# lucidrains/phenaki-pytorch

Hardware: NVIDIA H100
Metric: cvivit_encode_frames_per_s (higher is better)
Workload: dtype bf16

## Files before the change

phenaki_pytorch_b200/csrc/gemm_wgmma.cu:

```cuda
#include "phk_common.cuh"
#include "phk_sm90.cuh"
#include <mutex>
#include <unordered_map>

namespace phk {

constexpr int GM = 128;
constexpr int GN = 128;
constexpr int GK = 64;
constexpr int GSTAGES = 4;
constexpr int EPI_WARPS = 16;
constexpr int GTHREADS = 128 + EPI_WARPS * 32;
constexpr int STAGE_BYTES = GM * GK * 2;
constexpr int CPAD = 132;
constexpr int CSTAGE_BYTES = GM * CPAD * 4;
constexpr int RING_BYTES = GSTAGES * 2 * STAGE_BYTES;
constexpr int SMEM_TOTAL = RING_BYTES + CSTAGE_BYTES + 256  + 1024 ;

struct EpiParams {
  void* C; int64_t ldc; int64_t M; int N; int K;
  const float* bias; const float* residual;
  int64_t seg_len, seg_stride, seg_off;
  int m_tiles, n_tiles;
  int tma_epi;
  const float* nscale; int norm_cols; float nmul;
  alignas(64) CUtensorMap tmC;
};


__device__ __forceinline__ void epi_bar_sync() { asm volatile("bar.sync 1, %0;" ::"n"(EPI_WARPS * 32) : "memory"); }

template <bool BOX>
__device__ __forceinline__ void acc_to_stage(const float (&d)[32], uint8_t* stage, int rq, int cq, int w, int lane,
                                             bool add) {
  const int r0 = rq + 16 * w + (lane >> 2);
#pragma unroll
  for (int j = 0; j < 8; ++j) {
    const int c = cq + 8 * j + 2 * (lane & 3);
#pragma unroll
    for (int h = 0; h < 2; ++h) {
      const int r = r0 + 8 * h;
      float2* dst = BOX ? reinterpret_cast<float2*>(stage + (c >> 5) * (GM * 128) + r * 128 +
                                                    ((((c & 31) >> 2) ^ (r & 7)) << 4) + (c & 3) * 4)
                        : reinterpret_cast<float2*>(reinterpret_cast<float*>(stage) + r * CPAD + c);
      float2 v = make_float2(d[4 * j + 2 * h], d[4 * j + 2 * h + 1]);
      if (add) { const float2 o = *dst; v.x += o.x; v.y += o.y; }
      *dst = v;
    }
  }
}

__device__ __forceinline__ float geglu_fast(float g, float v) {
  const float g2 = fminf(g * g, 64.0f);
  float u = fmaf(g2, -0.00035151678851506f, 0.037005646021930225f);
  u = fmaf(u, g2, 0.7975078842858219f);
  float t;
  asm("tanh.approx.f32 %0, %1;" : "=f"(t) : "f"(g * u));
  const float h = 0.5f * (g * v);
  return fmaf(h, t, h);
}


template <int EPI>
__device__ __forceinline__ bool epi_residual_prefetch(const EpiParams& p, float* cstage, int64_t m0, int n0, int ew,
                                                      int lane) {
  const bool res_vec = EPI == 0 && p.residual && (p.ldc % 4 == 0) && (p.N % 4 == 0) &&
                       ((reinterpret_cast<uintptr_t>(p.residual) & 15) == 0);
  if (res_vec) {
    const int col = n0 + lane * 4;
    const uint32_t seg_len = (uint32_t)p.seg_len;
#pragma unroll 1
    for (int rb = 0; rb < GM / EPI_WARPS; rb += 8) {
      float4 rv[8];
#pragma unroll
      for (int u = 0; u < 8; ++u) {
        const int r = (rb + u) * EPI_WARPS + ew;
        const uint32_t m = (uint32_t)m0 + r;
        uint32_t orow = m;
        if (seg_len > 0) { const uint32_t q = m / seg_len; orow = q * (uint32_t)p.seg_stride + (uint32_t)p.seg_off + (m - q * seg_len); }
        rv[u] = make_float4(0.f, 0.f, 0.f, 0.f);
        if (m < (uint32_t)p.M && col < p.N) rv[u] = *reinterpret_cast<const float4*>(p.residual + (int64_t)orow * p.ldc + col);
      }
#pragma unroll
      for (int u = 0; u < 8; ++u)
        *reinterpret_cast<float4*>(cstage + ((rb + u) * EPI_WARPS + ew) * CPAD + lane * 4) = rv[u];
    }
    epi_bar_sync();
  }
  return res_vec;
}

__device__ __forceinline__ void tma_store_2d(const CUtensorMap* map, uint32_t src, int c0, int c1) {
  asm volatile("cp.async.bulk.tensor.2d.global.shared::cta.bulk_group [%0, {%2, %3}], [%1];"
               ::"l"(map), "r"(src), "r"(c0), "r"(c1)
               : "memory");
}
__device__ __forceinline__ void tma_store_commit() { asm volatile("cp.async.bulk.commit_group;" ::: "memory"); }
__device__ __forceinline__ void tma_store_wait_read() { asm volatile("cp.async.bulk.wait_group.read 0;" ::: "memory"); }
__device__ __forceinline__ void tma_store_wait_all() { asm volatile("cp.async.bulk.wait_group 0;" ::: "memory"); }

__device__ __forceinline__ void epi_tma_begin(const EpiParams& p, uint32_t stage_s, uint32_t bar_res, int m0, int n0,
                                              int ew, int lane) {
  const bool store_thread = ew == 0 && lane == 0;
  if (store_thread) tma_store_wait_read();
  epi_bar_sync();
  if (p.residual && store_thread) {
    mbar_expect_tx(bar_res, 4 * GM * 128);
#pragma unroll
    for (int c = 0; c < 4; ++c) tma_load_2d(&p.tmC, bar_res, stage_s + c * (GM * 128), n0 + 32 * c, m0);
  }
}
__device__ __forceinline__ void epi_tma_finish(const EpiParams& p, uint8_t* stage, uint32_t stage_s, int m0, int n0,
                                               int ew, int lg, int part, int lane) {
  const int r = lg * 32 + lane;
  float4* box_row = reinterpret_cast<float4*>(stage + part * (GM * 128) + r * 128);
  const int col0 = n0 + part * 32;
  const bool bias_vec = p.bias && (col0 + 31 < p.N) && ((reinterpret_cast<uintptr_t>(p.bias) & 15) == 0);
#pragma unroll
  for (int j = 0; j < 8; ++j) {
    const int pos = j ^ (r & 7);
    float4 o = box_row[pos];
    if (bias_vec) {
      const float4 bv = __ldg(reinterpret_cast<const float4*>(p.bias + col0) + j);
      o.x += bv.x; o.y += bv.y; o.z += bv.z; o.w += bv.w;
    } else if (p.bias) {
      const int c = col0 + 4 * j;
      if (c < p.N) o.x += __ldg(p.bias + c);
      if (c + 1 < p.N) o.y += __ldg(p.bias + c + 1);
      if (c + 2 < p.N) o.z += __ldg(p.bias + c + 2);
      if (c + 3 < p.N) o.w += __ldg(p.bias + c + 3);
    }
    box_row[pos] = o;
  }
  asm volatile("fence.proxy.async.shared::cta;" ::: "memory");
  epi_bar_sync();
  if (ew == 0 && lane == 0) {
#pragma unroll
    for (int c = 0; c < 4; ++c)
      if (n0 + 32 * c < p.N) tma_store_2d(&p.tmC, stage_s + c * (GM * 128), n0 + 32 * c, m0);
    tma_store_commit();
  }
}

template <int EPI>
__device__ __forceinline__ void epi_chunk(const EpiParams& p, float* cstage, int64_t m0, int n0, bool res_vec, int ew,
                                          int lane) {
  const uint32_t seg_len = (uint32_t)p.seg_len;
  constexpr int RPW = GM / EPI_WARPS;
  const int ncol0 = n0;
  const int nlim = p.N;
  if (EPI == 0) {
    const int col = ncol0 + lane * 4;
    const bool vec = (p.ldc % 4 == 0) && ((reinterpret_cast<uintptr_t>(p.C) & 15) == 0) && (col + 3 < nlim);
    float4 bv = make_float4(0.f, 0.f, 0.f, 0.f);
    if (p.bias) {
      if (col < nlim) bv.x = __ldg(p.bias + col);
      if (col + 1 < nlim) bv.y = __ldg(p.bias + col + 1);
      if (col + 2 < nlim) bv.z = __ldg(p.bias + col + 2);
      if (col + 3 < nlim) bv.w = __ldg(p.bias + col + 3);
    }
    const bool fast = (p.ldc % 4 == 0) && ((reinterpret_cast<uintptr_t>(p.C) & 15) == 0) && (p.N % 4 == 0) &&
                      (res_vec || !p.residual) && (m0 + GM <= p.M) && seg_len == 0;
    if (fast) {
      if (col < nlim) {
        float* cbase = reinterpret_cast<float*>(p.C) + (m0 + ew) * p.ldc + col;
        const float* sbase = cstage + ew * CPAD + lane * 4;
#pragma unroll 1
        for (int rb = 0; rb < RPW; rb += 8) {
          float4 o[8];
#pragma unroll
          for (int u = 0; u < 8; ++u) o[u] = *reinterpret_cast<const float4*>(sbase + (rb + u) * EPI_WARPS * CPAD);
#pragma unroll
          for (int u = 0; u < 8; ++u) {
            o[u].x += bv.x; o[u].y += bv.y; o[u].z += bv.z; o[u].w += bv.w;
            *reinterpret_cast<float4*>(cbase + (int64_t)(rb + u) * EPI_WARPS * p.ldc) = o[u];
          }
        }
      }
    } else
#pragma unroll 1
    for (int rb = 0; rb < RPW; rb += 8) {
      int64_t off[8];
      float4 rv[8];
#pragma unroll
      for (int u = 0; u < 8; ++u) {
        const int r = (rb + u) * EPI_WARPS + ew;
        const uint32_t m = (uint32_t)m0 + r;
        uint32_t orow = m;
        if (seg_len > 0) { const uint32_t q = m / seg_len; orow = q * (uint32_t)p.seg_stride + (uint32_t)p.seg_off + (m - q * seg_len); }
        off[u] = (m < (uint32_t)p.M && col < nlim) ? (int64_t)orow * p.ldc + col : -1;
        rv[u] = make_float4(0.f, 0.f, 0.f, 0.f);
        if (!res_vec && vec && p.residual && off[u] >= 0) rv[u] = *reinterpret_cast<const float4*>(p.residual + off[u]);
      }
#pragma unroll
      for (int u = 0; u < 8; ++u) {
        if (off[u] < 0) continue;
        const int r = (rb + u) * EPI_WARPS + ew;
        float4 o = *reinterpret_cast<const float4*>(cstage + r * CPAD + lane * 4);
        o.x += bv.x + rv[u].x; o.y += bv.y + rv[u].y; o.z += bv.z + rv[u].z; o.w += bv.w + rv[u].w;
        float* crow = reinterpret_cast<float*>(p.C) + off[u];
        if (vec) {
          *reinterpret_cast<float4*>(crow) = o;
        } else {
          const float ov[4] = {o.x, o.y, o.z, o.w};
          for (int j = 0; j < 4; ++j)
            if (col + j < nlim) crow[j] = ov[j] + ((p.residual && !res_vec) ? p.residual[off[u] + j] : 0.f);
        }
      }
    }
  } else if (EPI == 3) {
    const int col = ncol0 + lane * 4;
    const bool norm = ncol0 < p.norm_cols;
    float4 sc = make_float4(1.f, 1.f, 1.f, 1.f);
    if (norm) {
      const float4 t = __ldg(reinterpret_cast<const float4*>(p.nscale + ((lane * 4) & 63)));
      sc = make_float4(t.x * p.nmul, t.y * p.nmul, t.z * p.nmul, t.w * p.nmul);
    }
#pragma unroll 4
    for (int rr = 0; rr < RPW; ++rr) {
      const int r = rr * EPI_WARPS + ew;
      const uint32_t m = (uint32_t)m0 + r;
      float4 o = *reinterpret_cast<const float4*>(cstage + r * CPAD + lane * 4);
      if (norm) {
        float ss = o.x * o.x + o.y * o.y + o.z * o.z + o.w * o.w;
#pragma unroll
        for (int d = 8; d > 0; d >>= 1) ss += __shfl_xor_sync(0xffffffffu, ss, d);
        const float inv = 1.0f / fmaxf(sqrtf(ss), 1e-12f);
        o.x = (o.x * inv) * sc.x; o.y = (o.y * inv) * sc.y; o.z = (o.z * inv) * sc.z; o.w = (o.w * inv) * sc.w;
      }
      if (m < (uint32_t)p.M && col < nlim)
        *reinterpret_cast<uint2*>(reinterpret_cast<__nv_bfloat16*>(p.C) + (int64_t)m * p.ldc + col) =
            make_uint2(pack_bf16x2(o.x, o.y), pack_bf16x2(o.z, o.w));
    }
  } else {
    constexpr int CPL = 4;
    const int col = ncol0 + lane * CPL;
    float bv[CPL];
#pragma unroll
    for (int j = 0; j < CPL; ++j) bv[j] = (p.bias && col + j < nlim) ? __ldg(p.bias + col + j) : 0.f;
    const bool vec = (p.ldc % CPL == 0) && ((reinterpret_cast<uintptr_t>(p.C) & 15) == 0) && (col + CPL - 1 < nlim);
#pragma unroll 4
    for (int rr = 0; rr < RPW; ++rr) {
      const int r = rr * EPI_WARPS + ew;
      const uint32_t m = (uint32_t)m0 + r;
      if (m >= (uint32_t)p.M) break;
      int64_t orow = m;
      if (seg_len > 0) { const uint32_t q = m / seg_len; orow = q * (uint32_t)p.seg_stride + (uint32_t)p.seg_off + (m - q * seg_len); }
      float o[CPL];
#pragma unroll
      for (int j = 0; j < CPL; ++j) o[j] = cstage[r * CPAD + lane * CPL + j] + bv[j];
      __nv_bfloat16* crow = reinterpret_cast<__nv_bfloat16*>(p.C) + orow * p.ldc + col;
      if (vec) {
        *reinterpret_cast<uint2*>(crow) = make_uint2(pack_bf16x2(o[0], o[1]), pack_bf16x2(o[2], o[3]));
      } else {
#pragma unroll
        for (int j = 0; j < CPL; ++j)
          if (col + j < nlim) crow[j] = __float2bfloat16_rn(o[j]);
      }
    }
  }
  epi_bar_sync();
}

template <int EPI, bool DUAL>
__global__ void __launch_bounds__(GTHREADS, 1) gemm_bf16_kernel(const __grid_constant__ CUtensorMap tmA,
                                                                const __grid_constant__ CUtensorMap tmB,
                                                                const __grid_constant__ EpiParams p,
                                                                const __grid_constant__ CUtensorMap tmA2,
                                                                const __grid_constant__ CUtensorMap tmB2,
                                                                const __grid_constant__ EpiParams p2) {
  pdl_trigger();
  extern __shared__ uint8_t smem_raw[];
  const uint32_t base = (smem_u32(smem_raw) + 1023u) & ~1023u;
  uint8_t* base_ptr = smem_raw + (base - smem_u32(smem_raw));
  const uint32_t sA = base, sB = base + GSTAGES * STAGE_BYTES;
  float* cstage = reinterpret_cast<float*>(base_ptr + RING_BYTES);
  const uint32_t bars = base + RING_BYTES + CSTAGE_BYTES;
  const uint32_t bar_res = bars + 16 * GSTAGES;
  const int warp = threadIdx.x >> 5, lane = threadIdx.x & 31;
  const int tiles1 = p.m_tiles * p.n_tiles;
  const int num_tiles = tiles1 + (DUAL ? p2.m_tiles * p2.n_tiles : 0);
  const int my_tiles = (int)blockIdx.x < num_tiles ? (num_tiles - 1 - (int)blockIdx.x) / (int)gridDim.x + 1 : 0;
  auto tile_of = [&](int i, int& m0, int& n0) -> bool {
    int tile = (int)blockIdx.x + i * (int)gridDim.x;
    const bool second = DUAL && tile >= tiles1;
    if (second) tile -= tiles1;
    const int mt = second ? p2.m_tiles : p.m_tiles;
    m0 = (tile % mt) * GM;
    n0 = (tile / mt) * GN;
    return second;
  };
  auto kblocks = [&](bool second) { return ((second ? p2.K : p.K) + GK - 1) / GK; };

  if (threadIdx.x == 0) {
    asm volatile("prefetch.tensormap [%0];" ::"l"(&tmA) : "memory");
    asm volatile("prefetch.tensormap [%0];" ::"l"(&tmB) : "memory");
    if (DUAL) {
      asm volatile("prefetch.tensormap [%0];" ::"l"(&tmA2) : "memory");
      asm volatile("prefetch.tensormap [%0];" ::"l"(&tmB2) : "memory");
    }
    for (int s = 0; s < GSTAGES; ++s) {
      mbar_init(bars + 8 * s, 1);
      mbar_init(bars + 8 * (GSTAGES + s), EPI_WARPS);
    }
    mbar_init(bar_res, 1);
    asm volatile("fence.mbarrier_init.release.cluster;" ::: "memory");
  }
  __syncthreads();
  pdl_wait();

  if (warp < 4) {
    if (warp == 0 && lane == 0) {
      int stage = 0;
      uint32_t phase = 0;
      for (int it = 0; it < my_tiles; ++it) {
        int m0, n0;
        const bool second = tile_of(it, m0, n0);
        const int num_kb = kblocks(second);
        const CUtensorMap* ma = second ? &tmA2 : &tmA;
        const CUtensorMap* mb = second ? &tmB2 : &tmB;
        for (int kb = 0; kb < num_kb; ++kb) {
          mbar_wait(bars + 8 * (GSTAGES + stage), phase ^ 1);
          const uint32_t full = bars + 8 * stage;
          mbar_expect_tx(full, 2 * STAGE_BYTES);
          tma_load_2d(ma, full, sA + stage * STAGE_BYTES, kb * GK, m0);
          tma_load_2d(mb, full, sB + stage * STAGE_BYTES, kb * GK, n0);
          if (++stage == GSTAGES) { stage = 0; phase ^= 1; }
        }
      }
    }
  } else {
    const int ew = warp - 4;
    const int lg = warp & 3;
    const int part = ew >> 2;
    const int wg = ew >> 2;
    const int rq = (wg & 1) * 64, cq = (wg >> 1) * 64;
    uint32_t res_phase = 0;
    int stage = 0;
    uint32_t phase = 0;
    for (int it = 0; it < my_tiles; ++it) {
      int m0, n0;
      const bool second = tile_of(it, m0, n0);
      const EpiParams& pp = second ? p2 : p;
      const bool tma = EPI == 0 && pp.tma_epi;
      bool res_vec = false;
      if (tma) epi_tma_begin(pp, base + RING_BYTES, bar_res, m0, n0, ew, lane);
      else if (EPI == 0) res_vec = epi_residual_prefetch<EPI>(pp, cstage, m0, n0, ew, lane);
      else epi_bar_sync();
      float d[32];
#pragma unroll
      for (int i = 0; i < 32; ++i) d[i] = 0.f;
      const int num_kb = kblocks(second);
      for (int kb = 0; kb < num_kb; ++kb) {
        mbar_wait(bars + 8 * stage, phase);
        const uint64_t da = gmma_desc(sA + stage * STAGE_BYTES + rq * 128);
        const uint64_t db = gmma_desc(sB + stage * STAGE_BYTES + cq * 128);
        wgmma_fence();
#pragma unroll
        for (int k = 0; k < GK / 16; ++k)
          wgmma_m64n64k16_ss<0>(d, da + 2 * k, db + 2 * k, 1u);
        wgmma_commit();
        wgmma_wait<0>();
        __syncwarp();
        if (lane == 0) mbar_arrive(bars + 8 * (GSTAGES + stage));
        if (++stage == GSTAGES) { stage = 0; phase ^= 1; }
      }
      if (tma) {
        if (pp.residual) { mbar_wait(bar_res, res_phase); res_phase ^= 1; }
        acc_to_stage<true>(d, reinterpret_cast<uint8_t*>(cstage), rq, cq, ew & 3, lane, pp.residual != nullptr);
      } else {
        acc_to_stage<false>(d, reinterpret_cast<uint8_t*>(cstage), rq, cq, ew & 3, lane, res_vec);
      }
      epi_bar_sync();
      if (tma)
        epi_tma_finish(pp, reinterpret_cast<uint8_t*>(cstage), base + RING_BYTES, m0, n0, ew, lg, part, lane);
      else
        epi_chunk<EPI>(pp, cstage, m0, n0, res_vec, ew, lane);
    }
    if (EPI == 0 && ew == 0 && lane == 0) tma_store_wait_read();
  }
  __syncthreads();
}

constexpr int GG_STAGES = 6;
constexpr int GG_THREADS = 384;
constexpr int GG_PRODUCER_REGS = 40, GG_CONSUMER_REGS = 232;
constexpr int GG_SMEM_TOTAL = GG_STAGES * 2 * STAGE_BYTES + 128  + 1024 ;
constexpr int GG_BAR_TURN = 1;

__global__ void __launch_bounds__(GG_THREADS, 1) gemm_bf16_geglu_kernel(const __grid_constant__ CUtensorMap tmA,
                                                                        const __grid_constant__ CUtensorMap tmB,
                                                                        const __grid_constant__ EpiParams p) {
  pdl_trigger();
  extern __shared__ uint8_t smem_raw[];
  const uint32_t base = (smem_u32(smem_raw) + 1023u) & ~1023u;
  const uint32_t sA = base, sB = base + GG_STAGES * STAGE_BYTES;
  const uint32_t bars = base + GG_STAGES * 2 * STAGE_BYTES;
  const int warp = threadIdx.x >> 5, lane = threadIdx.x & 31;
  const int num_tiles = p.m_tiles * p.n_tiles;
  const int my_tiles = (int)blockIdx.x < num_tiles ? (num_tiles - 1 - (int)blockIdx.x) / (int)gridDim.x + 1 : 0;
  const int num_kb = (p.K + GK - 1) / GK;
  auto tile_of = [&](int i, int& m0, int& n0) {
    const int tile = (int)blockIdx.x + i * (int)gridDim.x;
    m0 = (tile % p.m_tiles) * GM;
    n0 = (tile / p.m_tiles) * GN;
  };

  if (threadIdx.x == 0) {
    asm volatile("prefetch.tensormap [%0];" ::"l"(&tmA) : "memory");
    asm volatile("prefetch.tensormap [%0];" ::"l"(&tmB) : "memory");
    for (int s = 0; s < GG_STAGES; ++s) {
      mbar_init(bars + 8 * s, 1);
      mbar_init(bars + 8 * (GG_STAGES + s), 4);
    }
    asm volatile("fence.mbarrier_init.release.cluster;" ::: "memory");
  }
  __syncthreads();
  pdl_wait();

  if (warp < 4) {
    setmaxnreg_dec<GG_PRODUCER_REGS>();
    if (warp == 0 && lane == 0) {
      int stage = 0;
      uint32_t phase = 0;
      for (int it = 0; it < my_tiles; ++it) {
        int m0, n0;
        tile_of(it, m0, n0);
        for (int kb = 0; kb < num_kb; ++kb) {
          mbar_wait(bars + 8 * (GG_STAGES + stage), phase ^ 1);
          const uint32_t full = bars + 8 * stage;
          mbar_expect_tx(full, 2 * STAGE_BYTES);
          tma_load_2d(&tmA, full, sA + stage * STAGE_BYTES, kb * GK, m0);
          tma_load_2d(&tmB, full, sB + stage * STAGE_BYTES, kb * GK, n0);
          if (++stage == GG_STAGES) { stage = 0; phase ^= 1; }
        }
      }
    }
  } else {
    setmaxnreg_inc<GG_CONSUMER_REGS>();
    const int wg = (warp >> 2) - 1;
    const int w = warp & 3;
    int stage = 0;
    uint32_t phase = 0;
    for (int it = 0; it < my_tiles; ++it) {
      if ((it & 1) != wg) {
        stage += num_kb;
        while (stage >= GG_STAGES) { stage -= GG_STAGES; phase ^= 1; }
        continue;
      }
      int m0, n0;
      tile_of(it, m0, n0);
      if (it > 0) named_bar_sync(GG_BAR_TURN + wg, 256);
      float acc[2][64];
      int prev = 0;
      for (int kb = 0; kb < num_kb; ++kb) {
        mbar_wait(bars + 8 * stage, phase);
        const uint64_t da0 = gmma_desc(sA + stage * STAGE_BYTES);
        const uint64_t da1 = gmma_desc(sA + stage * STAGE_BYTES + 64 * 128);
        const uint64_t db = gmma_desc(sB + stage * STAGE_BYTES);
        wgmma_fence();
#pragma unroll
        for (int k = 0; k < GK / 16; ++k) {
          const uint32_t accumulate = (kb > 0 || k > 0) ? 1u : 0u;
          wgmma_m64n128k16_ss(acc[0], da0 + 2 * k, db + 2 * k, accumulate);
          wgmma_m64n128k16_ss(acc[1], da1 + 2 * k, db + 2 * k, accumulate);
        }
        wgmma_commit();
        wgmma_wait<1>();
        if (kb > 0) {
          __syncwarp();
          if (lane == 0) mbar_arrive(bars + 8 * (GG_STAGES + prev));
        }
        prev = stage;
        if (++stage == GG_STAGES) { stage = 0; phase ^= 1; }
      }
      if (it + 1 < my_tiles) named_bar_arrive(GG_BAR_TURN + (wg ^ 1), 256);
      wgmma_wait<0>();
      __syncwarp();
      if (lane == 0) mbar_arrive(bars + 8 * (GG_STAGES + prev));
      __nv_bfloat16* C = reinterpret_cast<__nv_bfloat16*>(p.C);
      const int oc = n0 / 2 + 2 * (lane & 3);
#pragma unroll
      for (int r = 0; r < 4; ++r) {
        const uint32_t m = (uint32_t)m0 + 64 * (r >> 1) + 16 * w + (lane >> 2) + 8 * (r & 1);
        if (m >= (uint32_t)p.M) continue;
        int64_t orow = m;
        const uint32_t seg_len = (uint32_t)p.seg_len;
        if (seg_len > 0) { const uint32_t q = m / seg_len; orow = q * (uint32_t)p.seg_stride + (uint32_t)p.seg_off + (m - q * seg_len); }
        const float* a = acc[r >> 1] + 2 * (r & 1);
        uint32_t* crow = reinterpret_cast<uint32_t*>(C + orow * p.ldc + oc);
#pragma unroll
        for (int j = 0; j < 8; ++j)
          crow[4 * j] = pack_bf16x2(geglu_fast(a[4 * (j + 8)], a[4 * j]), geglu_fast(a[4 * (j + 8) + 1], a[4 * j + 1]));
      }
    }
  }
  __syncthreads();
}


struct MapKey {
  const void* ptr; int64_t rows, cols, ld; int box_rows;
  bool operator==(const MapKey& o) const {
    return ptr == o.ptr && rows == o.rows && cols == o.cols && ld == o.ld && box_rows == o.box_rows;
  }
};
struct MapKeyHash {
  size_t operator()(const MapKey& k) const {
    size_t h = std::hash<const void*>()(k.ptr);
    h = h * 1000003u ^ std::hash<int64_t>()(k.rows);
    h = h * 1000003u ^ std::hash<int64_t>()(k.cols);
    h = h * 1000003u ^ std::hash<int64_t>()(k.ld * 131 + k.box_rows);
    return h;
  }
};

static int get_tensor_map(const void* ptr, int64_t rows, int64_t cols, int64_t ld, int box_rows, CUtensorMap* out) {
  static std::unordered_map<MapKey, CUtensorMap, MapKeyHash> cache;
  static std::mutex mu;
  const MapKey key{ptr, rows, cols, ld, box_rows};
  std::lock_guard<std::mutex> lk(mu);
  auto it = cache.find(key);
  if (it != cache.end()) { *out = it->second; return 0; }
  EncodeTiledFn fn = encode_fn();
  PHK_REQUIRE(fn, PHK_E_UNSUPPORTED, "cuTensorMapEncodeTiled not available from the driver");
  const cuuint64_t gdim[2] = {(cuuint64_t)cols, (cuuint64_t)rows};
  const cuuint64_t gstride[1] = {(cuuint64_t)ld * 2};
  const cuuint32_t box[2] = {(cuuint32_t)GK, (cuuint32_t)box_rows};
  const cuuint32_t estr[2] = {1, 1};
  CUtensorMap m;
  const CUresult r = fn(&m, CU_TENSOR_MAP_DATA_TYPE_BFLOAT16, 2, const_cast<void*>(ptr), gdim, gstride, box, estr,
                        CU_TENSOR_MAP_INTERLEAVE_NONE, CU_TENSOR_MAP_SWIZZLE_128B, CU_TENSOR_MAP_L2_PROMOTION_L2_256B,
                        CU_TENSOR_MAP_FLOAT_OOB_FILL_NONE);
  PHK_REQUIRE(r == CUDA_SUCCESS, PHK_E_ARG, "cuTensorMapEncodeTiled rejected the operand (alignment / pitch)");
  if (cache.size() > 8192) cache.clear();
  cache.emplace(key, m);
  *out = m;
  return 0;
}

static int get_c_map(const void* ptr, int64_t rows, int64_t cols, int64_t ld, CUtensorMap* out) {
  static std::unordered_map<MapKey, CUtensorMap, MapKeyHash> cache;
  static std::mutex mu;
  const MapKey key{ptr, rows, cols, ld, -32};
  std::lock_guard<std::mutex> lk(mu);
  auto it = cache.find(key);
  if (it != cache.end()) { *out = it->second; return 0; }
  EncodeTiledFn fn = encode_fn();
  PHK_REQUIRE(fn, PHK_E_UNSUPPORTED, "cuTensorMapEncodeTiled not available from the driver");
  const cuuint64_t gdim[2] = {(cuuint64_t)cols, (cuuint64_t)rows};
  const cuuint64_t gstride[1] = {(cuuint64_t)ld * 4};
  const cuuint32_t box[2] = {32, (cuuint32_t)GM};
  const cuuint32_t estr[2] = {1, 1};
  CUtensorMap m;
  const CUresult r = fn(&m, CU_TENSOR_MAP_DATA_TYPE_FLOAT32, 2, const_cast<void*>(ptr), gdim, gstride, box, estr,
                        CU_TENSOR_MAP_INTERLEAVE_NONE, CU_TENSOR_MAP_SWIZZLE_128B, CU_TENSOR_MAP_L2_PROMOTION_L2_256B,
                        CU_TENSOR_MAP_FLOAT_OOB_FILL_NONE);
  PHK_REQUIRE(r == CUDA_SUCCESS, PHK_E_ARG, "cuTensorMapEncodeTiled rejected the output (alignment / pitch)");
  if (cache.size() > 8192) cache.clear();
  cache.emplace(key, m);
  *out = m;
  return 0;
}

static int maybe_tma_epilogue(EpiParams& p, int epilogue) {
  p.tma_epi = 0;
  if (epilogue != 0 || p.seg_len != 0 || p.ldc % 4 != 0 || (reinterpret_cast<uintptr_t>(p.C) & 15) != 0 ||
      (p.residual && p.residual != p.C))
    return 0;
  PHK_TRY(get_c_map(p.C, p.M, p.N, p.ldc, &p.tmC));
  p.tma_epi = 1;
  return 0;
}

template <int EPI>
static int launch_gemm(const CUtensorMap& ta, const CUtensorMap& tb, const EpiParams& p, cudaStream_t st) {
  static unsigned long long configured_mask = 0;
  const bool configured = device_configured(&configured_mask);
  if (!configured) {
    PHK_CUDA(cudaFuncSetAttribute(gemm_bf16_kernel<EPI, false>, cudaFuncAttributeMaxDynamicSharedMemorySize, SMEM_TOTAL));
    mark_configured(&configured_mask);
  }
  const int tiles = p.m_tiles * p.n_tiles;
  const int grid = tiles < kNumSMs ? tiles : kNumSMs;
  PHK_CUDA(launch_pdl(gemm_bf16_kernel<EPI, false>, dim3(grid), dim3(GTHREADS), (size_t)(SMEM_TOTAL), st, ta, tb, p, ta, tb, p));
  PHK_LAUNCH_CHECK();
  return 0;
}

static int launch_gemm_geglu(const CUtensorMap& ta, const CUtensorMap& tb, const EpiParams& p, cudaStream_t st) {
  static unsigned long long configured_mask = 0;
  if (!device_configured(&configured_mask)) {
    PHK_CUDA(cudaFuncSetAttribute(gemm_bf16_geglu_kernel, cudaFuncAttributeMaxDynamicSharedMemorySize, GG_SMEM_TOTAL));
    mark_configured(&configured_mask);
  }
  const int tiles = p.m_tiles * p.n_tiles;
  const int grid = tiles < kNumSMs ? tiles : kNumSMs;
  PHK_CUDA(launch_pdl(gemm_bf16_geglu_kernel, dim3(grid), dim3(GG_THREADS), (size_t)GG_SMEM_TOTAL, st, ta, tb, p));
  PHK_LAUNCH_CHECK();
  return 0;
}

template <int EPI>
static int launch_gemm_dual(const CUtensorMap& ta, const CUtensorMap& tb, const EpiParams& p, const CUtensorMap& ta2,
                            const CUtensorMap& tb2, const EpiParams& p2, cudaStream_t st) {
  static unsigned long long configured_mask = 0;
  const bool configured = device_configured(&configured_mask);
  if (!configured) {
    PHK_CUDA(cudaFuncSetAttribute(gemm_bf16_kernel<EPI, true>, cudaFuncAttributeMaxDynamicSharedMemorySize, SMEM_TOTAL));
    mark_configured(&configured_mask);
  }
  const int tiles = p.m_tiles * p.n_tiles + p2.m_tiles * p2.n_tiles;
  const int grid = tiles < kNumSMs ? tiles : kNumSMs;
  PHK_CUDA(launch_pdl(gemm_bf16_kernel<EPI, true>, dim3(grid), dim3(GTHREADS), (size_t)(SMEM_TOTAL), st, ta, tb, p, ta2, tb2, p2));
  PHK_LAUNCH_CHECK();
  return 0;
}

}

using namespace phk;

extern "C" int phk_gemm_bf16(const void* A, int64_t lda, const void* W, int64_t ldw, void* C, int64_t ldc, int64_t M,
                             int32_t N, int32_t K, const float* bias, const float* residual, int64_t seg_len,
                             int64_t seg_stride, int64_t seg_off, int32_t epilogue, phk_stream_t s) {
  Prof prof_(FAM_GEMM_BF16, s, 2.0 * (double)M * N * K);
  PHK_REQUIRE(A && W && C, PHK_E_ARG, "phk_gemm_bf16: null pointer");
  PHK_REQUIRE(M >= 0 && N > 0 && K > 0 && lda >= K && ldw >= K, PHK_E_ARG, "phk_gemm_bf16: bad size");
  PHK_REQUIRE(lda % 8 == 0 && ldw % 8 == 0 && (reinterpret_cast<uintptr_t>(A) & 15) == 0 &&
                  (reinterpret_cast<uintptr_t>(W) & 15) == 0,
              PHK_E_ARG, "phk_gemm_bf16: operands must be 16-byte aligned with leading dimensions multiple of 8 (TMA)");
  PHK_REQUIRE(epilogue >= 0 && epilogue <= 2, PHK_E_ARG, "phk_gemm_bf16: unknown epilogue");
  PHK_REQUIRE(epilogue != 2 || (N % 128 == 0 && !bias && !residual && ldc % 2 == 0 &&
                                (reinterpret_cast<uintptr_t>(C) & 3) == 0),
              PHK_E_ARG, "phk_gemm_bf16: GEGLU epilogue needs N % 128 == 0, an even ldc and no bias/residual");
  PHK_REQUIRE(M < (1LL << 31) - GM, PHK_E_UNSUPPORTED, "phk_gemm_bf16: M too large");
  if (M == 0) return 0;
  CUtensorMap ta, tb;
  PHK_TRY(get_tensor_map(A, M, K, lda, GM, &ta));
  cudaStream_t st = to_stream(s);
  PHK_TRY(get_tensor_map(W, N, K, ldw, GN, &tb));
  EpiParams p{C, ldc, M, N, K, bias, residual, seg_len, seg_stride, seg_off, (int)((M + GM - 1) / GM), (N + GN - 1) / GN};
  PHK_REQUIRE((int64_t)p.m_tiles * p.n_tiles < (1LL << 31), PHK_E_UNSUPPORTED, "phk_gemm_bf16: too many tiles");
  PHK_TRY(maybe_tma_epilogue(p, epilogue));
  if (epilogue == 2) return launch_gemm_geglu(ta, tb, p, st);
  if (epilogue == 1) return launch_gemm<1>(ta, tb, p, st);
  return launch_gemm<0>(ta, tb, p, st);
}

extern "C" int phk_gemm_bf16_x2(const void* A1, int64_t lda1, const void* W1, int64_t ldw1, float* C1, int64_t ldc1,
                                int64_t M1, int32_t N1, int32_t K1, const float* bias1, const void* A2, int64_t lda2,
                                const void* W2, int64_t ldw2, float* C2, int64_t ldc2, int64_t M2, int32_t N2,
                                int32_t K2, const float* bias2, phk_stream_t s) {
  Prof prof_(FAM_GEMM_BF16, s, 2.0 * ((double)M1 * N1 * K1 + (double)M2 * N2 * K2));
  PHK_REQUIRE(A1 && W1 && C1 && A2 && W2 && C2, PHK_E_ARG, "phk_gemm_bf16_x2: null pointer");
  PHK_REQUIRE(M1 > 0 && M2 > 0 && N1 > 0 && K1 > 0 && N2 > 0 && K2 > 0 && lda1 >= K1 && ldw1 >= K1 && lda2 >= K2 &&
                  ldw2 >= K2, PHK_E_ARG, "phk_gemm_bf16_x2: bad size");
  PHK_REQUIRE(lda1 % 8 == 0 && ldw1 % 8 == 0 && lda2 % 8 == 0 && ldw2 % 8 == 0 &&
                  ((reinterpret_cast<uintptr_t>(A1) | reinterpret_cast<uintptr_t>(W1) | reinterpret_cast<uintptr_t>(A2) |
                    reinterpret_cast<uintptr_t>(W2)) & 15) == 0,
              PHK_E_ARG, "phk_gemm_bf16_x2: operands must be 16-byte aligned with leading dimensions multiple of 8 (TMA)");
  PHK_REQUIRE(M1 < (1LL << 31) - 2 * GM && M2 < (1LL << 31) - 2 * GM, PHK_E_UNSUPPORTED, "phk_gemm_bf16_x2: M too large");
  CUtensorMap ta, tb, ta2, tb2;
  PHK_TRY(get_tensor_map(A1, M1, K1, lda1, GM, &ta));
  PHK_TRY(get_tensor_map(A2, M2, K2, lda2, GM, &ta2));
  PHK_TRY(get_tensor_map(W1, N1, K1, ldw1, GN, &tb));
  PHK_TRY(get_tensor_map(W2, N2, K2, ldw2, GN, &tb2));
  EpiParams p{C1, ldc1, M1, N1, K1, bias1, nullptr, 0, 0, 0, (int)((M1 + GM - 1) / GM), (N1 + GN - 1) / GN};
  EpiParams p2{C2, ldc2, M2, N2, K2, bias2, nullptr, 0, 0, 0, (int)((M2 + GM - 1) / GM), (N2 + GN - 1) / GN};
  PHK_REQUIRE((int64_t)p.m_tiles * p.n_tiles + (int64_t)p2.m_tiles * p2.n_tiles < (1LL << 31), PHK_E_UNSUPPORTED,
              "phk_gemm_bf16_x2: too many tiles");
  return launch_gemm_dual<0>(ta, tb, p, ta2, tb2, p2, to_stream(s));
}

extern "C" int phk_gemm_bf16_qkv(const void* xn, const void* xraw, int64_t lda, const void* Wq, const void* Wkv, int64_t ldw,
                                 void* Qn, void* KVn, int64_t M, int32_t I, int32_t K, const float* q_scale,
                                 const float* k_scale, float sim_scale, phk_stream_t s) {
  Prof prof_(FAM_GEMM_BF16, s, 2.0 * (double)M * 3.0 * I * K);
  PHK_REQUIRE(xn && xraw && Wq && Wkv && Qn && KVn && q_scale && k_scale, PHK_E_ARG, "phk_gemm_bf16_qkv: null pointer");
  PHK_REQUIRE(M > 0 && I > 0 && I % 128 == 0 && K > 0 && lda >= K && ldw >= K, PHK_E_ARG,
              "phk_gemm_bf16_qkv: heads * 64 must be a multiple of 128");
  PHK_REQUIRE(lda % 8 == 0 && ldw % 8 == 0 &&
                  ((reinterpret_cast<uintptr_t>(xn) | reinterpret_cast<uintptr_t>(xraw) | reinterpret_cast<uintptr_t>(Wq) |
                    reinterpret_cast<uintptr_t>(Wkv) | reinterpret_cast<uintptr_t>(q_scale) |
                    reinterpret_cast<uintptr_t>(k_scale)) & 15) == 0 &&
                  ((reinterpret_cast<uintptr_t>(Qn) | reinterpret_cast<uintptr_t>(KVn)) & 7) == 0,
              PHK_E_ARG, "phk_gemm_bf16_qkv: operands must be 16-byte aligned with leading dimensions multiple of 8 (TMA)");
  PHK_REQUIRE(M < (1LL << 31) - 2 * GM, PHK_E_UNSUPPORTED, "phk_gemm_bf16_qkv: M too large");
  CUtensorMap ta, tb, ta2, tb2;
  PHK_TRY(get_tensor_map(xn, M, K, lda, GM, &ta));
  PHK_TRY(get_tensor_map(xraw, M, K, lda, GM, &ta2));
  PHK_TRY(get_tensor_map(Wq, I, K, ldw, GN, &tb));
  PHK_TRY(get_tensor_map(Wkv, 2 * I, K, ldw, GN, &tb2));
  EpiParams p{Qn, I, M, I, K, nullptr, nullptr, 0, 0, 0, (int)((M + GM - 1) / GM), I / GN};
  EpiParams p2{KVn, 2 * (int64_t)I, M, 2 * I, K, nullptr, nullptr, 0, 0, 0, (int)((M + GM - 1) / GM), 2 * I / GN};
  p.tma_epi = 0; p.nscale = q_scale; p.norm_cols = I; p.nmul = sim_scale;
  p2.tma_epi = 0; p2.nscale = k_scale; p2.norm_cols = I; p2.nmul = 1.0f;
  PHK_REQUIRE((int64_t)p.m_tiles * p.n_tiles + (int64_t)p2.m_tiles * p2.n_tiles < (1LL << 31), PHK_E_UNSUPPORTED,
              "phk_gemm_bf16_qkv: too many tiles");
  return launch_gemm_dual<3>(ta, tb, p, ta2, tb2, p2, to_stream(s));
}

extern "C" int phk_gemm_bf16_qnorm(const void* xn, int64_t lda, const void* Wq, int64_t ldw, void* Qn, int64_t M, int32_t I,
                                   int32_t K, const float* q_scale, float sim_scale, phk_stream_t s) {
  Prof prof_(FAM_GEMM_BF16, s, 2.0 * (double)M * I * K);
  PHK_REQUIRE(xn && Wq && Qn && q_scale, PHK_E_ARG, "phk_gemm_bf16_qnorm: null pointer");
  PHK_REQUIRE(M > 0 && I > 0 && I % 128 == 0 && K > 0 && lda >= K && ldw >= K, PHK_E_ARG,
              "phk_gemm_bf16_qnorm: heads * 64 must be a multiple of 128");
  PHK_REQUIRE(lda % 8 == 0 && ldw % 8 == 0 &&
                  ((reinterpret_cast<uintptr_t>(xn) | reinterpret_cast<uintptr_t>(Wq) | reinterpret_cast<uintptr_t>(q_scale)) & 15) == 0 &&
                  (reinterpret_cast<uintptr_t>(Qn) & 7) == 0,
              PHK_E_ARG, "phk_gemm_bf16_qnorm: operands must be 16-byte aligned with leading dimensions multiple of 8 (TMA)");
  PHK_REQUIRE(M < (1LL << 31) - 2 * GM, PHK_E_UNSUPPORTED, "phk_gemm_bf16_qnorm: M too large");
  CUtensorMap ta, tb;
  PHK_TRY(get_tensor_map(xn, M, K, lda, GM, &ta));
  PHK_TRY(get_tensor_map(Wq, I, K, ldw, GN, &tb));
  EpiParams p{Qn, I, M, I, K, nullptr, nullptr, 0, 0, 0, (int)((M + GM - 1) / GM), I / GN};
  p.tma_epi = 0; p.nscale = q_scale; p.norm_cols = I; p.nmul = sim_scale;
  return launch_gemm<3>(ta, tb, p, to_stream(s));
}
```

Before: 116,900.

## Route dual-problem GEMMs through ping-pong warp-specialized kernel with register epilogues

Result: faster. 123,200, median of 6 (+5.4%).

```diff
diff --git a/phenaki_pytorch_b200/csrc/gemm_wgmma.cu b/phenaki_pytorch_b200/csrc/gemm_wgmma.cu
--- a/phenaki_pytorch_b200/csrc/gemm_wgmma.cu
+++ b/phenaki_pytorch_b200/csrc/gemm_wgmma.cu
@@ -59,6 +59,13 @@
   const float h = 0.5f * (g * v);
   return fmaf(h, t, h);
 }
+
+__device__ __forceinline__ float head_sumsq_first(float c0, float c1) { return __fmaf_rn(c0, c0, __fmul_rn(c1, c1)); }
+__device__ __forceinline__ float head_sumsq_next(float c2, float c3, float s) {
+  return __fmaf_rn(c3, c3, __fmaf_rn(c2, c2, s));
+}
+__device__ __forceinline__ float head_inv_norm(float ss) { return 1.0f / fmaxf(sqrtf(ss), 1e-12f); }
+__device__ __forceinline__ float head_scale(float c, float inv, float sc) { return __fmul_rn(__fmul_rn(c, inv), sc); }
 
 
 template <int EPI>
@@ -222,11 +229,12 @@
       const uint32_t m = (uint32_t)m0 + r;
       float4 o = *reinterpret_cast<const float4*>(cstage + r * CPAD + lane * 4);
       if (norm) {
-        float ss = o.x * o.x + o.y * o.y + o.z * o.z + o.w * o.w;
+        float ss = head_sumsq_next(o.z, o.w, head_sumsq_first(o.x, o.y));
 #pragma unroll
         for (int d = 8; d > 0; d >>= 1) ss += __shfl_xor_sync(0xffffffffu, ss, d);
-        const float inv = 1.0f / fmaxf(sqrtf(ss), 1e-12f);
-        o.x = (o.x * inv) * sc.x; o.y = (o.y * inv) * sc.y; o.z = (o.z * inv) * sc.z; o.w = (o.w * inv) * sc.w;
+        const float inv = head_inv_norm(ss);
+        o.x = head_scale(o.x, inv, sc.x); o.y = head_scale(o.y, inv, sc.y);
+        o.z = head_scale(o.z, inv, sc.z); o.w = head_scale(o.w, inv, sc.w);
       }
       if (m < (uint32_t)p.M && col < nlim)
         *reinterpret_cast<uint2*>(reinterpret_cast<__nv_bfloat16*>(p.C) + (int64_t)m * p.ldc + col) =
@@ -262,13 +270,8 @@
   epi_bar_sync();
 }
 
-template <int EPI, bool DUAL>
-__global__ void __launch_bounds__(GTHREADS, 1) gemm_bf16_kernel(const __grid_constant__ CUtensorMap tmA,
-                                                                const __grid_constant__ CUtensorMap tmB,
-                                                                const __grid_constant__ EpiParams p,
-                                                                const __grid_constant__ CUtensorMap tmA2,
-                                                                const __grid_constant__ CUtensorMap tmB2,
-                                                                const __grid_constant__ EpiParams p2) {
+template <int EPI>
+__device__ __forceinline__ void gemm_quadrant(const CUtensorMap& tmA, const CUtensorMap& tmB, const EpiParams& p) {
   pdl_trigger();
   extern __shared__ uint8_t smem_raw[];
   const uint32_t base = (smem_u32(smem_raw) + 1023u) & ~1023u;
@@ -277,6 +280,114 @@
   float* cstage = reinterpret_cast<float*>(base_ptr + RING_BYTES);
   const uint32_t bars = base + RING_BYTES + CSTAGE_BYTES;
   const uint32_t bar_res = bars + 16 * GSTAGES;
+  const int warp = threadIdx.x >> 5, lane = threadIdx.x & 31;
+  const int num_tiles = p.m_tiles * p.n_tiles;
+  const int my_tiles = (int)blockIdx.x < num_tiles ? (num_tiles - 1 - (int)blockIdx.x) / (int)gridDim.x + 1 : 0;
+  auto tile_of = [&](int i, int& m0, int& n0) {
+    const int tile = (int)blockIdx.x + i * (int)gridDim.x;
+    m0 = (tile % p.m_tiles) * GM;
+    n0 = (tile / p.m_tiles) * GN;
+  };
+  const int num_kb = (p.K + GK - 1) / GK;
+
+  if (threadIdx.x == 0) {
+    asm volatile("prefetch.tensormap [%0];" ::"l"(&tmA) : "memory");
+    asm volatile("prefetch.tensormap [%0];" ::"l"(&tmB) : "memory");
+    for (int s = 0; s < GSTAGES; ++s) {
+      mbar_init(bars + 8 * s, 1);
+      mbar_init(bars + 8 * (GSTAGES + s), EPI_WARPS);
+    }
+    mbar_init(bar_res, 1);
+    asm volatile("fence.mbarrier_init.release.cluster;" ::: "memory");
+  }
+  __syncthreads();
+  pdl_wait();
+
+  if (warp < 4) {
+    if (warp == 0 && lane == 0) {
+      int stage = 0;
+      uint32_t phase = 0;
+      for (int it = 0; it < my_tiles; ++it) {
+        int m0, n0;
+        tile_of(it, m0, n0);
+        for (int kb = 0; kb < num_kb; ++kb) {
+          mbar_wait(bars + 8 * (GSTAGES + stage), phase ^ 1);
+          const uint32_t full = bars + 8 * stage;
+          mbar_expect_tx(full, 2 * STAGE_BYTES);
+          tma_load_2d(&tmA, full, sA + stage * STAGE_BYTES, kb * GK, m0);
+          tma_load_2d(&tmB, full, sB + stage * STAGE_BYTES, kb * GK, n0);
+          if (++stage == GSTAGES) { stage = 0; phase ^= 1; }
+        }
+      }
+    }
+  } else {
+    const int ew = warp - 4;
+    const int lg = warp & 3;
+    const int part = ew >> 2;
+    const int wg = ew >> 2;
+    const int rq = (wg & 1) * 64, cq = (wg >> 1) * 64;
+    uint32_t res_phase = 0;
+    int stage = 0;
+    uint32_t phase = 0;
+    for (int it = 0; it < my_tiles; ++it) {
+      int m0, n0;
+      tile_of(it, m0, n0);
+      const bool tma = EPI == 0 && p.tma_epi;
+      bool res_vec = false;
+      if (tma) epi_tma_begin(p, base + RING_BYTES, bar_res, m0, n0, ew, lane);
+      else if (EPI == 0) res_vec = epi_residual_prefetch<EPI>(p, cstage, m0, n0, ew, lane);
+      else epi_bar_sync();
+      float d[32];
+#pragma unroll
+      for (int i = 0; i < 32; ++i) d[i] = 0.f;
+      for (int kb = 0; kb < num_kb; ++kb) {
+        mbar_wait(bars + 8 * stage, phase);
+        const uint64_t da = gmma_desc(sA + stage * STAGE_BYTES + rq * 128);
+        const uint64_t db = gmma_desc(sB + stage * STAGE_BYTES + cq * 128);
+        wgmma_fence();
+#pragma unroll
+        for (int k = 0; k < GK / 16; ++k)
+          wgmma_m64n64k16_ss<0>(d, da + 2 * k, db + 2 * k, 1u);
+        wgmma_commit();
+        wgmma_wait<0>();
+        __syncwarp();
+        if (lane == 0) mbar_arrive(bars + 8 * (GSTAGES + stage));
+        if (++stage == GSTAGES) { stage = 0; phase ^= 1; }
+      }
+      if (tma) {
+        if (p.residual) { mbar_wait(bar_res, res_phase); res_phase ^= 1; }
+        acc_to_stage<true>(d, reinterpret_cast<uint8_t*>(cstage), rq, cq, ew & 3, lane, p.residual != nullptr);
+      } else {
+        acc_to_stage<false>(d, reinterpret_cast<uint8_t*>(cstage), rq, cq, ew & 3, lane, res_vec);
+      }
+      epi_bar_sync();
+      if (tma)
+        epi_tma_finish(p, reinterpret_cast<uint8_t*>(cstage), base + RING_BYTES, m0, n0, ew, lg, part, lane);
+      else
+        epi_chunk<EPI>(p, cstage, m0, n0, res_vec, ew, lane);
+    }
+    if (EPI == 0 && ew == 0 && lane == 0) tma_store_wait_read();
+  }
+  __syncthreads();
+}
+
+constexpr int GG_STAGES = 6;
+constexpr int GG_THREADS = 384;
+constexpr int GG_PRODUCER_REGS = 40, GG_CONSUMER_REGS = 232;
+constexpr int GG_SMEM_TOTAL = GG_STAGES * 2 * STAGE_BYTES + 128  + 1024 ;
+constexpr int GG_BAR_TURN = 1;
+
+typedef float PingPongAcc[2][64];
+
+template <bool DUAL, class Epilogue>
+__device__ __forceinline__ void gemm_pingpong(const CUtensorMap& tmA, const CUtensorMap& tmB, const EpiParams& p,
+                                              const CUtensorMap& tmA2, const CUtensorMap& tmB2, const EpiParams& p2,
+                                              const Epilogue& epilogue) {
+  pdl_trigger();
+  extern __shared__ uint8_t smem_raw[];
+  const uint32_t base = (smem_u32(smem_raw) + 1023u) & ~1023u;
+  const uint32_t sA = base, sB = base + GG_STAGES * STAGE_BYTES;
+  const uint32_t bars = base + GG_STAGES * 2 * STAGE_BYTES;
   const int warp = threadIdx.x >> 5, lane = threadIdx.x & 31;
   const int tiles1 = p.m_tiles * p.n_tiles;
   const int num_tiles = tiles1 + (DUAL ? p2.m_tiles * p2.n_tiles : 0);
@@ -299,17 +410,17 @@
       asm volatile("prefetch.tensormap [%0];" ::"l"(&tmA2) : "memory");
       asm volatile("prefetch.tensormap [%0];" ::"l"(&tmB2) : "memory");
     }
-    for (int s = 0; s < GSTAGES; ++s) {
+    for (int s = 0; s < GG_STAGES; ++s) {
       mbar_init(bars + 8 * s, 1);
-      mbar_init(bars + 8 * (GSTAGES + s), EPI_WARPS);
-    }
-    mbar_init(bar_res, 1);
+      mbar_init(bars + 8 * (GG_STAGES + s), 4);
+    }
     asm volatile("fence.mbarrier_init.release.cluster;" ::: "memory");
   }
   __syncthreads();
   pdl_wait();
 
   if (warp < 4) {
+    setmaxnreg_dec<GG_PRODUCER_REGS>();
     if (warp == 0 && lane == 0) {
       int stage = 0;
       uint32_t phase = 0;
@@ -320,118 +431,11 @@
         const CUtensorMap* ma = second ? &tmA2 : &tmA;
         const CUtensorMap* mb = second ? &tmB2 : &tmB;
         for (int kb = 0; kb < num_kb; ++kb) {
-          mbar_wait(bars + 8 * (GSTAGES + stage), phase ^ 1);
+          mbar_wait(bars + 8 * (GG_STAGES + stage), phase ^ 1);
           const uint32_t full = bars + 8 * stage;
           mbar_expect_tx(full, 2 * STAGE_BYTES);
           tma_load_2d(ma, full, sA + stage * STAGE_BYTES, kb * GK, m0);
           tma_load_2d(mb, full, sB + stage * STAGE_BYTES, kb * GK, n0);
-          if (++stage == GSTAGES) { stage = 0; phase ^= 1; }
-        }
-      }
-    }
-  } else {
-    const int ew = warp - 4;
-    const int lg = warp & 3;
-    const int part = ew >> 2;
-    const int wg = ew >> 2;
-    const int rq = (wg & 1) * 64, cq = (wg >> 1) * 64;
-    uint32_t res_phase = 0;
-    int stage = 0;
-    uint32_t phase = 0;
-    for (int it = 0; it < my_tiles; ++it) {
-      int m0, n0;
-      const bool second = tile_of(it, m0, n0);
-      const EpiParams& pp = second ? p2 : p;
-      const bool tma = EPI == 0 && pp.tma_epi;
-      bool res_vec = false;
-      if (tma) epi_tma_begin(pp, base + RING_BYTES, bar_res, m0, n0, ew, lane);
-      else if (EPI == 0) res_vec = epi_residual_prefetch<EPI>(pp, cstage, m0, n0, ew, lane);
-      else epi_bar_sync();
-      float d[32];
-#pragma unroll
-      for (int i = 0; i < 32; ++i) d[i] = 0.f;
-      const int num_kb = kblocks(second);
-      for (int kb = 0; kb < num_kb; ++kb) {
-        mbar_wait(bars + 8 * stage, phase);
-        const uint64_t da = gmma_desc(sA + stage * STAGE_BYTES + rq * 128);
-        const uint64_t db = gmma_desc(sB + stage * STAGE_BYTES + cq * 128);
-        wgmma_fence();
-#pragma unroll
-        for (int k = 0; k < GK / 16; ++k)
-          wgmma_m64n64k16_ss<0>(d, da + 2 * k, db + 2 * k, 1u);
-        wgmma_commit();
-        wgmma_wait<0>();
-        __syncwarp();
-        if (lane == 0) mbar_arrive(bars + 8 * (GSTAGES + stage));
-        if (++stage == GSTAGES) { stage = 0; phase ^= 1; }
-      }
-      if (tma) {
-        if (pp.residual) { mbar_wait(bar_res, res_phase); res_phase ^= 1; }
-        acc_to_stage<true>(d, reinterpret_cast<uint8_t*>(cstage), rq, cq, ew & 3, lane, pp.residual != nullptr);
-      } else {
-        acc_to_stage<false>(d, reinterpret_cast<uint8_t*>(cstage), rq, cq, ew & 3, lane, res_vec);
-      }
-      epi_bar_sync();
-      if (tma)
-        epi_tma_finish(pp, reinterpret_cast<uint8_t*>(cstage), base + RING_BYTES, m0, n0, ew, lg, part, lane);
-      else
-        epi_chunk<EPI>(pp, cstage, m0, n0, res_vec, ew, lane);
-    }
-    if (EPI == 0 && ew == 0 && lane == 0) tma_store_wait_read();
-  }
-  __syncthreads();
-}
-
-constexpr int GG_STAGES = 6;
-constexpr int GG_THREADS = 384;
-constexpr int GG_PRODUCER_REGS = 40, GG_CONSUMER_REGS = 232;
-constexpr int GG_SMEM_TOTAL = GG_STAGES * 2 * STAGE_BYTES + 128  + 1024 ;
-constexpr int GG_BAR_TURN = 1;
-
-__global__ void __launch_bounds__(GG_THREADS, 1) gemm_bf16_geglu_kernel(const __grid_constant__ CUtensorMap tmA,
-                                                                        const __grid_constant__ CUtensorMap tmB,
-                                                                        const __grid_constant__ EpiParams p) {
-  pdl_trigger();
-  extern __shared__ uint8_t smem_raw[];
-  const uint32_t base = (smem_u32(smem_raw) + 1023u) & ~1023u;
-  const uint32_t sA = base, sB = base + GG_STAGES * STAGE_BYTES;
-  const uint32_t bars = base + GG_STAGES * 2 * STAGE_BYTES;
-  const int warp = threadIdx.x >> 5, lane = threadIdx.x & 31;
-  const int num_tiles = p.m_tiles * p.n_tiles;
-  const int my_tiles = (int)blockIdx.x < num_tiles ? (num_tiles - 1 - (int)blockIdx.x) / (int)gridDim.x + 1 : 0;
-  const int num_kb = (p.K + GK - 1) / GK;
-  auto tile_of = [&](int i, int& m0, int& n0) {
-    const int tile = (int)blockIdx.x + i * (int)gridDim.x;
-    m0 = (tile % p.m_tiles) * GM;
-    n0 = (tile / p.m_tiles) * GN;
-  };
-
-  if (threadIdx.x == 0) {
-    asm volatile("prefetch.tensormap [%0];" ::"l"(&tmA) : "memory");
-    asm volatile("prefetch.tensormap [%0];" ::"l"(&tmB) : "memory");
-    for (int s = 0; s < GG_STAGES; ++s) {
-      mbar_init(bars + 8 * s, 1);
-      mbar_init(bars + 8 * (GG_STAGES + s), 4);
-    }
-    asm volatile("fence.mbarrier_init.release.cluster;" ::: "memory");
-  }
-  __syncthreads();
-  pdl_wait();
-
-  if (warp < 4) {
-    setmaxnreg_dec<GG_PRODUCER_REGS>();
-    if (warp == 0 && lane == 0) {
-      int stage = 0;
-      uint32_t phase = 0;
-      for (int it = 0; it < my_tiles; ++it) {
-        int m0, n0;
-        tile_of(it, m0, n0);
-        for (int kb = 0; kb < num_kb; ++kb) {
-          mbar_wait(bars + 8 * (GG_STAGES + stage), phase ^ 1);
-          const uint32_t full = bars + 8 * stage;
-          mbar_expect_tx(full, 2 * STAGE_BYTES);
-          tma_load_2d(&tmA, full, sA + stage * STAGE_BYTES, kb * GK, m0);
-          tma_load_2d(&tmB, full, sB + stage * STAGE_BYTES, kb * GK, n0);
           if (++stage == GG_STAGES) { stage = 0; phase ^= 1; }
         }
       }
@@ -443,15 +447,16 @@
     int stage = 0;
     uint32_t phase = 0;
     for (int it = 0; it < my_tiles; ++it) {
+      int m0, n0;
+      const bool second = tile_of(it, m0, n0);
+      const int num_kb = kblocks(second);
       if ((it & 1) != wg) {
         stage += num_kb;
         while (stage >= GG_STAGES) { stage -= GG_STAGES; phase ^= 1; }
         continue;
       }
-      int m0, n0;
-      tile_of(it, m0, n0);
       if (it > 0) named_bar_sync(GG_BAR_TURN + wg, 256);
-      float acc[2][64];
+      PingPongAcc acc;
       int prev = 0;
       for (int kb = 0; kb < num_kb; ++kb) {
         mbar_wait(bars + 8 * stage, phase);
@@ -478,24 +483,134 @@
       wgmma_wait<0>();
       __syncwarp();
       if (lane == 0) mbar_arrive(bars + 8 * (GG_STAGES + prev));
-      __nv_bfloat16* C = reinterpret_cast<__nv_bfloat16*>(p.C);
-      const int oc = n0 / 2 + 2 * (lane & 3);
-#pragma unroll
-      for (int r = 0; r < 4; ++r) {
-        const uint32_t m = (uint32_t)m0 + 64 * (r >> 1) + 16 * w + (lane >> 2) + 8 * (r & 1);
-        if (m >= (uint32_t)p.M) continue;
-        int64_t orow = m;
-        const uint32_t seg_len = (uint32_t)p.seg_len;
-        if (seg_len > 0) { const uint32_t q = m / seg_len; orow = q * (uint32_t)p.seg_stride + (uint32_t)p.seg_off + (m - q * seg_len); }
-        const float* a = acc[r >> 1] + 2 * (r & 1);
-        uint32_t* crow = reinterpret_cast<uint32_t*>(C + orow * p.ldc + oc);
-#pragma unroll
-        for (int j = 0; j < 8; ++j)
-          crow[4 * j] = pack_bf16x2(geglu_fast(a[4 * (j + 8)], a[4 * j]), geglu_fast(a[4 * (j + 8) + 1], a[4 * j + 1]));
-      }
+      epilogue(second ? p2 : p, acc, m0, n0, w, lane);
     }
   }
   __syncthreads();
+}
+
+struct GegluEpilogue {
+  __device__ __forceinline__ void operator()(const EpiParams& p, const PingPongAcc& acc, int m0, int n0, int w,
+                                             int lane) const {
+    __nv_bfloat16* C = reinterpret_cast<__nv_bfloat16*>(p.C);
+    const int oc = n0 / 2 + 2 * (lane & 3);
+#pragma unroll
+    for (int r = 0; r < 4; ++r) {
+      const uint32_t m = (uint32_t)m0 + 64 * (r >> 1) + 16 * w + (lane >> 2) + 8 * (r & 1);
+      if (m >= (uint32_t)p.M) continue;
+      int64_t orow = m;
+      const uint32_t seg_len = (uint32_t)p.seg_len;
+      if (seg_len > 0) { const uint32_t q = m / seg_len; orow = q * (uint32_t)p.seg_stride + (uint32_t)p.seg_off + (m - q * seg_len); }
+      const float* a = acc[r >> 1] + 2 * (r & 1);
+      uint32_t* crow = reinterpret_cast<uint32_t*>(C + orow * p.ldc + oc);
+#pragma unroll
+      for (int j = 0; j < 8; ++j)
+        crow[4 * j] = pack_bf16x2(geglu_fast(a[4 * (j + 8)], a[4 * j]), geglu_fast(a[4 * (j + 8) + 1], a[4 * j + 1]));
+    }
+  }
+};
+
+struct QkNormEpilogue {
+  __device__ __forceinline__ void operator()(const EpiParams& p, const PingPongAcc& acc, int m0, int n0, int w,
+                                             int lane) const {
+    const int t = lane & 3;
+    const bool norm = n0 < p.norm_cols;
+    float2 sc[8];
+#pragma unroll
+    for (int jj = 0; jj < 8; ++jj) sc[jj] = make_float2(1.f, 1.f);
+    if (norm) {
+#pragma unroll
+      for (int jj = 0; jj < 8; ++jj) {
+        const float2 s = __ldg(reinterpret_cast<const float2*>(p.nscale + 8 * jj + 2 * t));
+        sc[jj] = make_float2(s.x * p.nmul, s.y * p.nmul);
+      }
+    }
+    __nv_bfloat16* C = reinterpret_cast<__nv_bfloat16*>(p.C);
+#pragma unroll
+    for (int r = 0; r < 4; ++r) {
+      const uint32_t m = (uint32_t)m0 + 64 * (r >> 1) + 16 * w + (lane >> 2) + 8 * (r & 1);
+      const float* a = acc[r >> 1] + 2 * (r & 1);
+      uint32_t* crow = reinterpret_cast<uint32_t*>(C + (int64_t)m * p.ldc + n0 + 2 * t);
+#pragma unroll
+      for (int hd = 0; hd < 2; ++hd) {
+        float inv = 1.f;
+        if (norm) {
+          float s[8];
+#pragma unroll
+          for (int jj = 0; jj < 8; ++jj) {
+            const float c0 = a[4 * (8 * hd + jj)], c1 = a[4 * (8 * hd + jj) + 1];
+            const float first = __shfl_xor_sync(0xffffffffu, head_sumsq_first(c0, c1), 1);
+            s[jj] = head_sumsq_next(c0, c1, first);
+          }
+          float ss = ((s[0] + s[4]) + (s[2] + s[6])) + ((s[1] + s[5]) + (s[3] + s[7]));
+          ss += __shfl_xor_sync(0xffffffffu, ss, 2);
+          ss = __shfl_sync(0xffffffffu, ss, lane | 1);
+          inv = head_inv_norm(ss);
+        }
+        if (m < (uint32_t)p.M) {
+#pragma unroll
+          for (int jj = 0; jj < 8; ++jj) {
+            float x = a[4 * (8 * hd + jj)], y = a[4 * (8 * hd + jj) + 1];
+            if (norm) { x = head_scale(x, inv, sc[jj].x); y = head_scale(y, inv, sc[jj].y); }
+            crow[4 * (8 * hd + jj)] = pack_bf16x2(x, y);
+          }
+        }
+      }
+    }
+  }
+};
+
+struct Fp32BiasEpilogue {
+  __device__ __forceinline__ void operator()(const EpiParams& p, const PingPongAcc& acc, int m0, int n0, int w,
+                                             int lane) const {
+    const int c0 = n0 + 2 * (lane & 3);
+    float2 bv[16];
+#pragma unroll
+    for (int j = 0; j < 16; ++j) {
+      const int c = c0 + 8 * j;
+      bv[j].x = (p.bias && c < p.N) ? __ldg(p.bias + c) : 0.f;
+      bv[j].y = (p.bias && c + 1 < p.N) ? __ldg(p.bias + c + 1) : 0.f;
+    }
+    const bool vec = (p.ldc % 2 == 0) && ((reinterpret_cast<uintptr_t>(p.C) & 7) == 0);
+#pragma unroll
+    for (int r = 0; r < 4; ++r) {
+      const uint32_t m = (uint32_t)m0 + 64 * (r >> 1) + 16 * w + (lane >> 2) + 8 * (r & 1);
+      if (m >= (uint32_t)p.M) continue;
+      const float* a = acc[r >> 1] + 2 * (r & 1);
+      float* crow = reinterpret_cast<float*>(p.C) + (int64_t)m * p.ldc + c0;
+#pragma unroll
+      for (int j = 0; j < 16; ++j) {
+        const float2 o = make_float2(a[4 * j] + bv[j].x, a[4 * j + 1] + bv[j].y);
+        const int c = c0 + 8 * j;
+        if (vec && c + 1 < p.N) {
+          *reinterpret_cast<float2*>(crow + 8 * j) = o;
+        } else {
+          if (c < p.N) crow[8 * j] = o.x;
+          if (c + 1 < p.N) crow[8 * j + 1] = o.y;
+        }
+      }
+    }
+  }
+};
+
+__global__ void __launch_bounds__(GG_THREADS, 1) gemm_bf16_geglu_kernel(const __grid_constant__ CUtensorMap tmA,
+                                                                        const __grid_constant__ CUtensorMap tmB,
+                                                                        const __grid_constant__ EpiParams p) {
+  gemm_pingpong<false>(tmA, tmB, p, tmA, tmB, p, GegluEpilogue{});
+}
+
+template <int EPI, bool DUAL>
+__global__ void __launch_bounds__(DUAL ? GG_THREADS : GTHREADS, 1) gemm_bf16_kernel(
+    const __grid_constant__ CUtensorMap tmA, const __grid_constant__ CUtensorMap tmB, const __grid_constant__ EpiParams p,
+    const __grid_constant__ CUtensorMap tmA2, const __grid_constant__ CUtensorMap tmB2,
+    const __grid_constant__ EpiParams p2) {
+  if constexpr (DUAL) {
+    static_assert(EPI == 0 || EPI == 3, "two-problem launches have the fp32 (+bias) or the q/k,v epilogue");
+    if constexpr (EPI == 3) gemm_pingpong<true>(tmA, tmB, p, tmA2, tmB2, p2, QkNormEpilogue{});
+    else gemm_pingpong<true>(tmA, tmB, p, tmA2, tmB2, p2, Fp32BiasEpilogue{});
+  } else {
+    gemm_quadrant<EPI>(tmA, tmB, p);
+  }
 }
 
 
@@ -607,12 +722,12 @@
   static unsigned long long configured_mask = 0;
   const bool configured = device_configured(&configured_mask);
   if (!configured) {
-    PHK_CUDA(cudaFuncSetAttribute(gemm_bf16_kernel<EPI, true>, cudaFuncAttributeMaxDynamicSharedMemorySize, SMEM_TOTAL));
+    PHK_CUDA(cudaFuncSetAttribute(gemm_bf16_kernel<EPI, true>, cudaFuncAttributeMaxDynamicSharedMemorySize, GG_SMEM_TOTAL));
     mark_configured(&configured_mask);
   }
   const int tiles = p.m_tiles * p.n_tiles + p2.m_tiles * p2.n_tiles;
   const int grid = tiles < kNumSMs ? tiles : kNumSMs;
-  PHK_CUDA(launch_pdl(gemm_bf16_kernel<EPI, true>, dim3(grid), dim3(GTHREADS), (size_t)(SMEM_TOTAL), st, ta, tb, p, ta2, tb2, p2));
+  PHK_CUDA(launch_pdl(gemm_bf16_kernel<EPI, true>, dim3(grid), dim3(GG_THREADS), (size_t)GG_SMEM_TOTAL, st, ta, tb, p, ta2, tb2, p2));
   PHK_LAUNCH_CHECK();
   return 0;
 }
```
